# j4n1k/rl4co-slap

Hardware: AMD Instinct MI355X
Metric: env-steps/sec (batch×decode) SLAP & TSP-100 at 1/2/4/8 MI355X (higher is better)
Workload: dtype u8+i64+f32

## Files before the change

### rl4co_slap_amd/csrc/co_common.hpp

```cpp
#pragma once

#include <hip/hip_runtime.h>
#include <stdint.h>

#include "../../include/co_env.h"

namespace co {

constexpr int kWave = 64;

__device__ __forceinline__ int lane_id() { return threadIdx.x & (kWave - 1); }
__device__ __forceinline__ int wave_in_block() {
  return __builtin_amdgcn_readfirstlane(threadIdx.x >> 6);
}

template <typename T>
__device__ __forceinline__ T wave_sum(T v) {
#pragma unroll
  for (int off = 32; off > 0; off >>= 1) v += __shfl_xor(v, off, kWave);
  return v;
}

__device__ __forceinline__ float wave_max(float v) {
#pragma unroll
// ... 81 lines not shown
    const auto r = __builtin_amdgcn_permlane16_swap(v, v, false, false);
    v = op(r[0], r[1]);
  }
  if (RL >= 64) {
    const auto r = __builtin_amdgcn_permlane32_swap(v, v, false, false);
    v = op(r[0], r[1]);
  }
  return v;
}

template <int RL>
__device__ __forceinline__ double grp_sum_f64(double v) {
  uint32_t lo = (uint32_t)__double_as_longlong(v), hi = (uint32_t)(__double_as_longlong(v) >> 32);
  auto join = [](uint32_t l, uint32_t h) {
    return __longlong_as_double((long long)(((uint64_t)h << 32) | l));
  };
#define CO_DPP_F64(C)                                   \
  {                                                     \
    v = v + join(dpp_u<C>(lo), dpp_u<C>(hi));           \
    lo = (uint32_t)__double_as_longlong(v);             \
    hi = (uint32_t)(__double_as_longlong(v) >> 32);     \
  }
  if (RL >= 2) CO_DPP_F64(0xB1);
  if (RL >= 4) CO_DPP_F64(0x4E);
  if (RL >= 8) CO_DPP_F64(0x141);
  if (RL >= 16) CO_DPP_F64(0x140);
#undef CO_DPP_F64
  if (RL >= 32) {
    const auto rl = __builtin_amdgcn_permlane16_swap(lo, lo, false, false);
    const auto rh = __builtin_amdgcn_permlane16_swap(hi, hi, false, false);
    v = join(rl[0], rh[0]) + join(rl[1], rh[1]);
    lo = (uint32_t)__double_as_longlong(v);
    hi = (uint32_t)(__double_as_longlong(v) >> 32);
  }
  if (RL >= 64) {
    const auto rl = __builtin_amdgcn_permlane32_swap(lo, lo, false, false);
    const auto rh = __builtin_amdgcn_permlane32_swap(hi, hi, false, false);
    v = join(rl[0], rh[0]) + join(rl[1], rh[1]);
  }
  return v;
}

template <int RL>
__device__ __forceinline__ float grp_max(float v) {
  return __uint_as_float(grp_reduce<RL>(__float_as_uint(v), [](uint32_t x, uint32_t y) {
    return __float_as_uint(fmaxf(__uint_as_float(x), __uint_as_float(y)));
  }));
}
template <int RL>
__device__ __forceinline__ float grp_max_ord(float v) {
  const int b = __float_as_int(v);
  int o = b ^ ((b >> 31) & 0x7fffffff);
  o = (int)grp_reduce<RL>((uint32_t)o, [](uint32_t x, uint32_t y) {
    return (uint32_t)max((int)x, (int)y);
  });
  return __int_as_float(o ^ ((o >> 31) & 0x7fffffff));
}
template <int RL>
__device__ __forceinline__ float grp_sum(float v) {
  return __uint_as_float(grp_reduce<RL>(__float_as_uint(v), [](uint32_t x, uint32_t y) {
    return __float_as_uint(__uint_as_float(x) + __uint_as_float(y));
  }));
}
template <int RL>
__device__ __forceinline__ void grp_argmax(float& v, int& idx) {
  uint32_t uv = __float_as_uint(v), ui = (uint32_t)idx;
  grp_reduce2<RL>(uv, ui, [](uint32_t ov, uint32_t oi, uint32_t cv, uint32_t ci) {
    return argmax_better(__uint_as_float(ov), (int)oi, __uint_as_float(cv), (int)ci);
  });
  v = __uint_as_float(uv);
  idx = (int)ui;
}
template <int RL>
__device__ __forceinline__ int grp_min_int(int v) {
  return (int)grp_reduce<RL>((uint32_t)v, [](uint32_t x, uint32_t y) {
    return (uint32_t)min((int)x, (int)y);
  });
}
template <int RL>
__device__ __forceinline__ int grp_max_int(int v) {
  return (int)grp_reduce<RL>((uint32_t)v, [](uint32_t x, uint32_t y) {
    return (uint32_t)max((int)x, (int)y);
  });
}

template <int RL>
__device__ __forceinline__ void grp_argmin(float& v, int& idx) {
  uint32_t uv = __float_as_uint(v), ui = (uint32_t)idx;
  grp_reduce2<RL>(uv, ui, [](uint32_t ov, uint32_t oi, uint32_t cv, uint32_t ci) {
    const float a = __uint_as_float(ov), b = __uint_as_float(cv);
    return a < b || (a == b && (int)oi < (int)ci);
  });
  v = __uint_as_float(uv);
  idx = (int)ui;
}

template <int RL>
__device__ __forceinline__ void grp_argmin_split(float& v, int& idx) {
  const float m = __uint_as_float(grp_reduce<RL>(__float_as_uint(v), [](uint32_t a, uint32_t b) {
    return __float_as_uint(fminf(__uint_as_float(a), __uint_as_float(b)));
  }));
  const int cand = v == m ? idx : 0x7fffffff;
  idx = (int)grp_reduce<RL>((uint32_t)cand, [](uint32_t a, uint32_t b) {
    return (uint32_t)min((int)a, (int)b);
  });
  v = m;
}

struct StripMove {
  int i, j;
};

__device__ __forceinline__ StripMove strip_move(int q, int c, int n) {
  const int r = q + 1, a = n - r;
  const bool first = c < a;
  const int d = first ? r : n - 1 - r, t = first ? c : c - a;
  StripMove m;
  m.i = 1 + t;
  m.j = 1 + t + d;
  return m;
}

constexpr uint32_t kDistKeyInf = 0xff800000u;
__device__ __forceinline__ uint32_t dist_key(float d) {
  const uint32_t u = __float_as_uint(d + 0.0f);
  return u ^ ((uint32_t)((int32_t)u >> 31) | 0x80000000u);
}
__device__ __forceinline__ uint32_t key_sel32(uint64_t m, uint32_t t, uint32_t f) {
  uint32_t r;
  asm("v_cndmask_b32_e64 %0, %1, %2, %3" : "=v"(r) : "v"(f), "v"(t), "s"(m));
  return r;
}
__device__ __forceinline__ void key_cswap(uint64_t& a, uint64_t& b) {
  const uint64_t lt = __builtin_amdgcn_ballot_w64(a < b);
  const uint32_t alo = (uint32_t)a, ahi = (uint32_t)(a >> 32), blo = (uint32_t)b,
                 bhi = (uint32_t)(b >> 32);
  a = ((uint64_t)key_sel32(lt, ahi, bhi) << 32) | key_sel32(lt, alo, blo);
  b = ((uint64_t)key_sel32(lt, bhi, ahi) << 32) | key_sel32(lt, blo, alo);
}
template <int E>
__device__ __forceinline__ void sort_keys(uint64_t (&k)[E]) {
  static_assert((E & (E - 1)) == 0, "E must be a power of two");
#pragma unroll
  for (int p = 1; p < E; p <<= 1)
#pragma unroll
    for (int q = p; q > 0; q >>= 1)
#pragma unroll
      for (int j = q % p; j + q < E; j += 2 * q)
#pragma unroll
        for (int i = 0; i < q; ++i)
          if (i + j + q < E && (i + j) / (2 * p) == (i + j + q) / (2 * p))
            key_cswap(k[i + j], k[i + j + q]);
}

typedef __attribute__((address_space(3))) void lds_void;

template <int AUX = 0>
__device__ __forceinline__ void stage_bytes_lds(const unsigned char* __restrict__ src, int nbytes,
                                                unsigned char* dst) {
  const int lane = threadIdx.x & 63, wave = wave_in_block(), nw = blockDim.x >> 6;
  const int n16 = nbytes & ~15;
  for (int base = wave * 1024; base < n16; base += nw * 1024) {
    const int off = base + lane * 16;
    if (off < n16)
      __builtin_amdgcn_global_load_lds((const void*)(src + off), (lds_void*)(dst + base), 16, 0,
                                       AUX);
  }
  for (int k = n16 + (int)threadIdx.x; k < nbytes; k += blockDim.x) dst[k] = src[k];
  __builtin_amdgcn_s_waitcnt(0);
  __syncthreads();
}

template <int AUX = 0>
__device__ __forceinline__ void wave_dma(const unsigned char* __restrict__ src, int nbytes,
                                         unsigned char* dst) {
  const int lane = lane_id(), n16 = nbytes & ~15;
  for (int base = 0; base < n16; base += 1024) {
    if (base + lane * 16 < n16)
      __builtin_amdgcn_global_load_lds((const void*)(src + base + lane * 16),
                                       (lds_void*)(dst + base), 16, 0, AUX);
  }
  if (lane < ((nbytes - n16) >> 2))
    reinterpret_cast<uint32_t*>(dst + n16)[lane] = reinterpret_cast<const uint32_t*>(src + n16)[lane];
}

__device__ __forceinline__ void wave_dma_wait() {
  __builtin_amdgcn_s_waitcnt(0);
  __builtin_amdgcn_fence(__ATOMIC_RELEASE, "wavefront");
  __builtin_amdgcn_wave_barrier();
  __builtin_amdgcn_fence(__ATOMIC_ACQUIRE, "wavefront");
}

namespace {
__global__ void zero_i32_kernel(int32_t* p) { *p = 0; }
}
inline int zero_i32(int32_t* p, hipStream_t s) {
  hipLaunchKernelGGL(zero_i32_kernel, dim3(1), dim3(1), 0, s, p);
  return (int)hipGetLastError();
}

inline unsigned grid_for(int64_t work_items, int per_block, int64_t cap = 256 * 16) {
  int64_t g = (work_items + per_block - 1) / per_block;
  if (g < 1) g = 1;
  if (g > cap) g = cap;
  return (unsigned)g;
}

constexpr int64_t kMaxCoverThreads = ((int64_t)1 << 32) - 1;
inline unsigned cover_grid(int64_t work_items, int per_block, int block_threads = 256) {
  int64_t g = (work_items + per_block - 1) / per_block;
  if (g < 1) g = 1;
  if (g * (int64_t)block_threads > kMaxCoverThreads) return 0;
  return (unsigned)g;
}

inline int launch_status() {
  hipError_t e = hipGetLastError();
  return e == hipSuccess ? CO_OK : (int)e;
}

}

int co_internal_tsp_reward_stepmajor(int64_t B, int64_t N, const float* locs,
                                     int64_t locs_batch, const int64_t* acts, int64_t st,
                                     int check, float* reward, int32_t* status, void* stream);
int co_internal_tsp_reward_rows(int64_t B, int64_t N, const float* locs, int64_t locs_batch,
                                const int64_t* acts, int64_t sb, int check, float* reward,
                                int32_t* status, void* stream);
int co_internal_tsp_nearest_rollout(int64_t B, int64_t N, const float* locs, int64_t* acts_out,
                                    uint8_t* mask_out, int64_t* first_out, int64_t* cur_out,
                                    int64_t* i_out, uint8_t* done_out, uint8_t* step_reward_out,
                                    float* reward_out, void* stream);
```

### rl4co_slap_amd/csrc/co_diag.hpp

```cpp
#pragma once

namespace co {

#ifdef CO_DIAG_FASTTANH
constexpr bool kDiagFastTanh = true;
#else
constexpr bool kDiagFastTanh = false;
#endif

#ifdef CO_DIAG_FASTEXP
constexpr bool kDiagFastExp = true;
#else
constexpr bool kDiagFastExp = false;
#endif

#ifdef CO_DIAG_CERT_COUNT
constexpr bool kDiagCertCount = true;
#else
constexpr bool kDiagCertCount = false;
#endif

#ifdef CO_DIAG_CVRP_CUT
constexpr int kDiagCvrpCut = CO_DIAG_CVRP_CUT;
#else
constexpr int kDiagCvrpCut = 0;
#endif

constexpr bool kDiagTimingCut = kDiagFastTanh || kDiagFastExp || kDiagCvrpCut != 0;

}
```

### rl4co_slap_amd/csrc/decode_step.hip

```cpp
#include "decode_common.hpp"

#if defined(CO_DIAG_FASTTANH) || defined(CO_DIAG_FASTEXP) || defined(CO_DIAG_CVRP_CUT) || \
    defined(CO_DIAG_CERT_COUNT)
extern "C" __attribute__((visibility("default"))) const int co_variant_timing_cut_decode = 1;
#endif

extern "C" int co_decode_step_ex(int64_t B, int64_t N, const float* logits, int64_t lstride,
                                 const uint8_t* mask, float clip, float temp, int top_k,
                                 double top_p, int mode, const int64_t* action_in,
                                 int64_t* action_out, float* logp_sel, float* full, uint64_t seed,
                                 uint64_t offset, int32_t* status, void* stream) {
  if (B < 0 || N <= 0 || N > (1 << 24) || top_k < 0 || top_p < 0.0 || top_p > 1.0)
    return CO_E_INVAL;
  const bool cert = (mode & CO_DECODE_CERTIFIED) != 0 && (mode & CO_DECODE_FAST) == 0;
  const bool fast = (mode & CO_DECODE_FAST) != 0;
  mode &= ~(CO_DECODE_FAST | CO_DECODE_CERTIFIED);
  if (mode < 0 || mode > 2) return CO_E_MODE;
  if (B == 0) return CO_OK;
  if (!logits || !action_out) return CO_E_INVAL;
  if (mode == CO_DECODE_EVALUATE && !action_in) return CO_E_INVAL;
  hipStream_t s = (hipStream_t)stream;
  if (N > 64 * 32) {
    if (top_p > 0.0 && top_p < 1.0) return CO_E_INVAL;
    const dim3 lgrid((unsigned)(B < 65536 ? B : 65536)), lblock(kLongThreads);
    const int opt = (clip > 0.f ? kOptClip : 0) | (temp != 1.f ? kOptTemp : 0);
#define CO_LONG(O)                                                                             \
  hipLaunchKernelGGL(decode_long_kernel<O>, lgrid, lblock, 0, s, B, (int)N, logits, lstride,   \
                     mask, clip, temp, mode, action_in, action_out, logp_sel, full, seed, offset, \
                     status, top_k)
    switch (opt) {
      case 0: CO_LONG(0); break;
      case 1: CO_LONG(1); break;
      case 2: CO_LONG(2); break;
      default: CO_LONG(3);
    }
#undef CO_LONG
    return launch_status();
  }
  const dim3 grid(decode_grid(B, (int)N)), block(256);
  if (grid.x == 0) return CO_E_INVAL;
  const bool filtered = (top_k > 0 && top_k < N) || (top_p > 0.0 && top_p < 1.0);
  if (mode == CO_DECODE_GREEDY && !filtered) {
#define CO_GREEDY(RL, EPL, V)                                                                  \
  CO_OPT_DISPATCH_G(hipLaunchKernelGGL, (decode_greedy_kernel<RL, (EPL < 4 ? 4 : EPL), V, OPT>), \
                  grid, block, 0, s, B, (int)N, logits, lstride, mask, clip, temp, action_out,  \
                  logp_sel, full, status)
    switch (greedy_vw(N, lstride, logits, mask, mask, full)) {
      case 4: CO_ROW_DISPATCH(CO_GREEDY, 4); break;
      case 2: CO_GREEDY(CO_RL16, 16 / CO_RL16, 2); break;
      default: CO_ROW_DISPATCH(CO_GREEDY, 3);
    }
#undef CO_GREEDY
    return launch_status();
  }
#define CO_DECODE(RL, EPL, V)                                                                  \
  CO_OPT_DISPATCH(hipLaunchKernelGGL, (decode_kernel<RL, EPL, V, OPT>), grid, block, 0, s, B,   \
                  (int)N, logits, lstride, mask, clip, temp, mode, action_in, action_out,      \
                  logp_sel, full, seed, offset, status, top_k, top_p)
  if (decode_vec_ok(logits, lstride, mask, N)) {
    CO_ROW_DISPATCH(CO_DECODE, true);
  } else {
    CO_ROW_DISPATCH(CO_DECODE, false);
  }
#undef CO_DECODE
  return launch_status();
}

extern "C" int co_decode_step(int64_t B, int64_t N, const float* logits, int64_t lstride,
                              const uint8_t* mask, float clip, float temp, int mode,
                              const int64_t* action_in, int64_t* action_out, float* logp_sel,
                              float* full, uint64_t seed, uint64_t offset, int32_t* status,
                              void* stream) {
  return co_decode_step_ex(B, N, logits, lstride, mask, clip, temp, 0, 0.0, mode, action_in,
                           action_out, logp_sel, full, seed, offset, status, stream);
}

namespace {
__global__ __launch_bounds__(64) void beam_select_kernel(
    int64_t B, int BW, int N, const float* __restrict__ logp, int64_t lstride,
    const float* __restrict__ parent, const uint8_t* __restrict__ mask,
    int64_t* __restrict__ selected, int32_t* __restrict__ beam_parent,
    int64_t* __restrict__ beam_row, float* __restrict__ score_out, int32_t* status) {
  extern __shared__ __attribute__((aligned(16))) unsigned char smem[];
  const int T = BW * N;
  float* sc = reinterpret_cast<float*>(smem);
  uint32_t* taken = reinterpret_cast<uint32_t*>(sc + T);
  const int lane = threadIdx.x;
  for (int64_t b = blockIdx.x; b < B; b += gridDim.x) {
    for (int t = lane; t < T; t += 64) {
      const int s = t / N, c = t - s * N;
      const int64_t r = (int64_t)s * B + b;
      sc[t] = logp[r * lstride + c] + parent[r];
    }
    for (int w = lane; w < (T + 31) / 32; w += 64) taken[w] = 0u;
    __syncthreads();
    bool bad = false;
    for (int j = 0; j < BW; ++j) {
      float bv = -__builtin_inff();
      int bi = 0x7fffffff;
      for (int t = lane; t < T; t += 64) {
        const bool free_t = !((taken[t >> 5] >> (t & 31)) & 1u);
        const float v = sc[t];
        if (free_t && (bi == 0x7fffffff || argmax_better(v, t, bv, bi))) {
          bv = v;
          bi = t;
        }
      }
      wave_argmax(bv, bi);
      if (bi == 0x7fffffff) bi = 0;
      const int s = bi / N, c = bi - s * N;
      if (lane == 0) {
        taken[bi >> 5] |= 1u << (bi & 31);
        const int64_t row = (int64_t)j * B + b;
        selected[row] = c;
        beam_parent[row] = s;
        beam_row[row] = b + (int64_t)s * B;
        score_out[row] = bv;
        if (mask && !mask[(b + (int64_t)s * B) * N + c]) bad = true;
      }
      __syncthreads();
    }
    if (bad) set_status(status, CO_ST_INFEASIBLE);
    __syncthreads();
  }
}
}

extern "C" int co_beam_select(int64_t B, int64_t BW, int64_t N, const float* logp,
                              int64_t lstride, const float* parent, const uint8_t* mask,
                              int64_t* selected, int32_t* beam_parent, int64_t* beam_row,
                              float* score_out, int32_t* status, void* stream) {
  if (B < 0 || BW <= 0 || N <= 0 || BW > N * BW || BW * N > 36 * 1024) return CO_E_INVAL;
  if (B == 0) return CO_OK;
  if (!logp || !parent || !selected || !beam_parent || !beam_row || !score_out ||
      (mask && !status))
    return CO_E_INVAL;
  const int T = (int)(BW * N);
  const size_t shmem = (size_t)T * 4 + (size_t)((T + 31) / 32) * 4;
  if (shmem > 64 * 1024)
    (void)hipFuncSetAttribute((const void*)beam_select_kernel,
                              hipFuncAttributeMaxDynamicSharedMemorySize, (int)shmem);
  hipLaunchKernelGGL(beam_select_kernel, dim3((unsigned)(B < 65536 ? B : 65536)), dim3(64),
                     shmem, (hipStream_t)stream, B, (int)BW, (int)N, logp, lstride, parent,
                     mask, selected, beam_parent, beam_row, score_out, status);
  return launch_status();
}
```

### rl4co_slap_amd/csrc/rollout.hip

```cpp
#include "co_common.hpp"

using namespace co;

namespace {


inline int NW_launch(int64_t n) {
  const int w = (int)((n + 63) / 64);
  return w <= 1 ? 1 : (w == 2 ? 2 : 4);
}

template <int NW>
__device__ __forceinline__ void mask_row_to_lds(const uint64_t (&m)[NW], int n,
                                                unsigned char* row, int c_lo = 0,
                                                int c_hi = -1) {
  if (c_hi < 0) c_hi = n;
  if ((n & 3) == 0 && (c_lo & 3) == 0) {
    for (int c = c_lo; c < c_hi; c += 4) {
      uint32_t v = 0;
#pragma unroll
      for (int j = 0; j < 4; ++j) {
        const int cc = c + j;
        uint64_t w = 0;
#pragma unroll
        for (int k = 0; k < NW; ++k)
          if ((cc >> 6) == k) w = m[k];
        v |= (uint32_t)((w >> (cc & 63)) & 1ull) << (8 * j);
      }
      *reinterpret_cast<uint32_t*>(row + c) = v;
    }
  } else {
    for (int c = c_lo; c < c_hi; ++c) {
      uint64_t w = 0;
#pragma unroll
      for (int k = 0; k < NW; ++k)
        if ((c >> 6) == k) w = m[k];
      row[c] = (unsigned char)((w >> (c & 63)) & 1ull);
    }
  }
}

__device__ __forceinline__ void copy_tile_out(const unsigned char* scratch, int nbytes,
                                              uint8_t* __restrict__ dst) {
  const int tid = threadIdx.x;
  const int n16 = ((reinterpret_cast<uintptr_t>(dst) & 15) == 0) ? (nbytes & ~15) : 0;
  for (int off = tid * 16; off < n16; off += blockDim.x * 16)
    *reinterpret_cast<uint4*>(dst + off) = *reinterpret_cast<const uint4*>(scratch + off);
  for (int k = n16 + tid; k < nbytes; k += blockDim.x) dst[k] = scratch[k];
}

__device__ __forceinline__ void zero_tile_out(int nbytes, uint8_t* __restrict__ dst) {
  const int tid = threadIdx.x;
  const int n16 = ((reinterpret_cast<uintptr_t>(dst) & 15) == 0) ? (nbytes & ~15) : 0;
  for (int off = tid * 16; off < n16; off += blockDim.x * 16)
    *reinterpret_cast<uint4*>(dst + off) = make_uint4(0u, 0u, 0u, 0u);
  for (int k = n16 + tid; k < nbytes; k += blockDim.x) dst[k] = 0;
}

__host__ __device__ inline size_t tsp_tile_bytes(int N, int Q) {
  const size_t xy = (size_t)64 * N * 8;
  const size_t scr = (((size_t)64 * N + 15) & ~(size_t)15) + (size_t)Q * 64 * 8 + 64 * 8 + 64 * 4 +
                     16 * 4;
  return ((xy > scr ? xy : scr) + 15) & ~(size_t)15;
}

#ifndef CO_TEACH_Q
#define CO_TEACH_Q 4
#endif
#ifndef CO_TEACH_U
#define CO_TEACH_U 8
#endif
template <int NW, int Q, bool STATE, int NB = 0>
__global__ __launch_bounds__(64 * Q) void tsp_teacher_kernel(
    int64_t B, int N, const float2* __restrict__ locs, int64_t LB,
    const int64_t* __restrict__ acts_in, uint8_t* __restrict__ mask_out,
    int64_t* __restrict__ first_out, int64_t* __restrict__ cur_out, int64_t* __restrict__ i_out,
    uint8_t* __restrict__ done_out, uint8_t* __restrict__ step_reward_out,
    float* __restrict__ reward_out, int check, int32_t* status) {
  extern __shared__ __attribute__((aligned(16))) unsigned char smem[];
  float2* s_xy = reinterpret_cast<float2*>(smem);
  constexpr int VS = 2 * NW + 1;
  uint32_t* s_vis = reinterpret_cast<uint32_t*>(smem + tsp_tile_bytes(N, Q));
  const int lane = threadIdx.x & 63, q = wave_in_block();
  const int64_t row0 = (int64_t)blockIdx.x * 64;
  const int rows = (int)((B - row0) < 64 ? (B - row0) : 64);
  const int64_t b = row0 + lane;
  const bool live = lane < rows;

  const int R = (N - 1 + Q - 1) / Q;
  const int t_lo = 1 + q * R < N ? 1 + q * R : N;
  const int t_hi = t_lo + R < N ? t_lo + R : N;
  constexpr int U = CO_TEACH_U;
  int64_t bufA[U], bufB[U];
  const int64_t* ap = acts_in + (live ? b : row0);
  auto load = [&](int64_t (&dst)[U], int t0) {
    const int tc = t0 + U <= t_hi ? t0 : t_hi - U;
    const int64_t* p = ap + (int64_t)tc * B;
#pragma unroll
    for (int u = 0; u < U; ++u) {
      dst[u] = *p;
      p += B;
    }
  };
  const int nfull = (t_hi - t_lo) / U;
  const int64_t a_prev = ap[(int64_t)(q == 0 ? 0 : t_lo - 1) * B];
  if (nfull > 0) load(bufA, t_lo);
  if (q == 0) {
    for (int k = 0; k < NW; ++k) {
      const int lo = k * 64;
      const uint64_t w = (N >= lo + 64) ? ~0ull : (N > lo ? ((1ull << (N - lo)) - 1ull) : 0ull);
      s_vis[lane * VS + 2 * k] = (uint32_t)w;
      s_vis[lane * VS + 2 * k + 1] = (uint32_t)(w >> 32);
    }
  }
  stage_bytes_lds(reinterpret_cast<const unsigned char*>(locs + (row0 % LB) * N), rows * N * 8,
                  reinterpret_cast<unsigned char*>(s_xy));
  const float2* xy = s_xy + lane * N;
  uint32_t* vw = s_vis + lane * VS;
  uint32_t badw = 0;
  int a = 0;
  float px = 0.f, py = 0.f, fx = 0.f, fy = 0.f;
  double len = 0.0;
  if (live) {
    const uint32_t lo = (uint32_t)a_prev;
    const uint32_t in = ((uint32_t)(a_prev >> 32) == 0u) & (lo < (uint32_t)N);
    a = in ? (int)lo : 0;
    if (q == 0) {
      badw |= in ^ 1u;
      __hip_atomic_fetch_and(&vw[a >> 5], ~(1u << (a & 31)), __ATOMIC_RELAXED,
                             __HIP_MEMORY_SCOPE_WORKGROUP);
    }
    const float2 p0 = xy[a];
    px = fx = p0.x;
    py = fy = p0.y;
    auto run = [&](const int64_t (&src)[U], int cnt) {
      int av[U];
#pragma unroll
      for (int u = 0; u < U; ++u) {
        if (u < cnt) {
          const uint32_t l32 = (uint32_t)src[u];
          const uint32_t ok = ((uint32_t)(src[u] >> 32) == 0u) & (l32 < (uint32_t)N);
          badw |= ok ^ 1u;
          av[u] = ok ? (int)l32 : 0;
        }
      }
      float2 qq[U];
#pragma unroll
      for (int u = 0; u < U; ++u)
        if (u < cnt) qq[u] = xy[av[u]];
#pragma unroll
      for (int u = 0; u < U; ++u)
        if (u < cnt)
          __hip_atomic_fetch_and(&vw[av[u] >> 5], ~(1u << (av[u] & 31)), __ATOMIC_RELAXED,
// ... 150 lines not shown
#pragma unroll
      for (int k = 0; k < EPL; k += 2) {
        if (valid && t0 + k + 1 < N) {
          const longlong2 v = *reinterpret_cast<const longlong2*>(arow + t0 + k);
          av[k] = v.x;
          av[k + 1] = v.y;
        } else {
          av[k] = (valid && t0 + k < N) ? arow[t0 + k] : 0;
          av[k + 1] = 0;
        }
      }
    } else {
#pragma unroll
      for (int k = 0; k < EPL; ++k) av[k] = (valid && t0 + k < N) ? arow[t0 + k] : 0;
    }
    for (int j = sl; j < NWB; j += G) bits[j] = 0u;
    uint32_t bad = 0;
    int node[EPL];
#pragma unroll
    for (int k = 0; k < EPL; ++k) {
      const uint32_t l32 = (uint32_t)av[k];
      const bool ok = ((uint32_t)(av[k] >> 32) == 0u) & (l32 < (uint32_t)N);
      const bool in = t0 + k < N;
      bad |= (in && !ok) ? 1u : 0u;
      node[k] = ok ? (int)l32 : 0;
    }
    const float2* lrow = DMA ? s_xy + grp * N : locs + (LB == B ? rr : rr % LB) * (int64_t)N;
    float2 p[EPL];
    if constexpr (DMA) {
#pragma unroll
      for (int k = 0; k < EPL; ++k) p[k] = lrow[node[k]];
    } else {
#pragma unroll
      for (int k = 0; k < EPL; ++k)
        p[k] = (valid && t0 + k < N) ? lrow[node[k]] : make_float2(0.f, 0.f);
    }
    __builtin_amdgcn_fence(__ATOMIC_RELEASE, "wavefront");
    __builtin_amdgcn_wave_barrier();
    __builtin_amdgcn_fence(__ATOMIC_ACQUIRE, "wavefront");
#pragma unroll
    for (int k = 0; k < EPL; ++k)
      __hip_atomic_fetch_or(&bits[node[k] >> 5],
                            (valid && t0 + k < N) ? 1u << (node[k] & 31) : 0u, __ATOMIC_RELAXED,
                            __HIP_MEMORY_SCOPE_WAVEFRONT);
    double acc = 0.0;
#pragma unroll
    for (int k = 1; k < EPL; ++k) {
      const float dx = p[k].x - p[k - 1].x, dy = p[k].y - p[k - 1].y;
      const float e = __builtin_amdgcn_sqrtf(dx * dx + dy * dy);
      acc += t0 + k < N ? (double)e : 0.0;
    }
    const float nx = __shfl_down(p[0].x, 1, G), ny = __shfl_down(p[0].y, 1, G);
    const float fx = __shfl(p[0].x, 0, G), fy = __shfl(p[0].y, 0, G);
    const int tl = N - 1 - t0;
    float lx = p[EPL - 1].x, ly = p[EPL - 1].y;
#pragma unroll
    for (int k = 0; k < EPL - 1; ++k)
      if (k == tl) {
        lx = p[k].x;
        ly = p[k].y;
      }
    {
      const bool cross = t0 + EPL < N, closing = !cross && tl >= 0 && tl < EPL;
      const float tx = cross ? nx : fx, ty = cross ? ny : fy;
      const float dx = tx - lx, dy = ty - ly;
      const float e = __builtin_amdgcn_sqrtf(dx * dx + dy * dy);
      acc += (cross || closing) ? (double)e : 0.0;
    }
    const float len = (float)grp_sum_f64<G>(acc);
    __builtin_amdgcn_fence(__ATOMIC_RELEASE, "wavefront");
    __builtin_amdgcn_wave_barrier();
    __builtin_amdgcn_fence(__ATOMIC_ACQUIRE, "wavefront");
    int cnt = 0;
    for (int j = sl; j < nwords; j += G) cnt += __popc(bits[j]);
    cnt = (int)grp_reduce<G>((uint32_t)cnt, [](uint32_t x, uint32_t y) { return x + y; });
    bad = grp_reduce<G>(bad, [](uint32_t x, uint32_t y) { return x | y; });
    const bool full = cnt == N;
    if (check && valid && sl == 0 && (bad || !full)) set_status(status, CO_ST_INVALID_TOUR);
    if (!valid) return;
    if constexpr (STATE) {
      uint8_t* mrow = mask_out + r * (int64_t)N;
      const bool wide = ((reinterpret_cast<uintptr_t>(mrow) | (uintptr_t)N) & 3) == 0;
      if (wide) {
        for (int c4 = sl; c4 < (N >> 2); c4 += G) {
          uint32_t v = 0;
          if (!full) {
            const uint32_t nib = ~(bits[c4 >> 3] >> (4 * (c4 & 7))) & 0xfu;
            v = (nib & 1u) | ((nib & 2u) << 7) | ((nib & 4u) << 14) | ((nib & 8u) << 21);
          }
          __builtin_nontemporal_store(v, reinterpret_cast<uint32_t*>(mrow + 4 * c4));
        }
      } else {
        for (int c = sl; c < N; c += G)
          mrow[c] = full ? 0 : (uint8_t)(((bits[c >> 5] >> (c & 31)) & 1u) ^ 1u);
      }
      const int last_lane = (N - 1) / EPL;
      int lastnode = node[0];
#pragma unroll
      for (int k = 0; k < EPL; ++k)
        if (k == tl) lastnode = node[k];
      if (sl == 0) {
        first_out[r] = node[0];
        i_out[r] = N;
        reward_out[r] = -(float)len;
      }
      if (sl == last_lane) cur_out[r] = lastnode;
      if (sl == (G > 2 ? 2 : 1) % G) {
        done_out[r] = full;
        step_reward_out[r] = 0;
      }
    } else {
      if (sl == 0) reward_out[r] = -(float)len;
    }
  }
}

__device__ __forceinline__ float edge_len_hw(float x0, float y0, float x1, float y1) {
  const float dx = x1 - x0, dy = y1 - y0;
  return __builtin_amdgcn_sqrtf(dx * dx + dy * dy);
}
__device__ __forceinline__ int slap_pick_loc(int pp, const int32_t* asg, int L, bool& range) {
  const bool neg = pp < 0;
  int64_t loc = asg[neg ? 0 : pp];
  loc = loc < 0 ? loc + L : loc;
  const bool bad = neg || loc < 0 || loc >= L;
  range |= bad;
  return bad ? 0 : (int)loc;
}
template <int KU, typename PK>
__device__ __forceinline__ float slap_order_len(const PK* pk, const int32_t* asg,
                                                const float2* xy, int L, bool& range,
                                                int K = KU) {
  int pp[KU], lc[KU];
  float2 q[KU];
#pragma unroll
  for (int k = 0; k < KU; ++k) pp[k] = k < K ? pk[k] : 0;
#pragma unroll
  for (int k = 0; k < KU; ++k) lc[k] = k < K ? slap_pick_loc(pp[k], asg, L, range) : 0;
#pragma unroll
  for (int k = 0; k < KU; ++k) q[k] = xy[lc[k]];
  float len = 0.f;
#pragma unroll
  for (int k = 1; k < KU; ++k)
    if (k < K) len += edge_len_hw(q[k - 1].x, q[k - 1].y, q[k].x, q[k].y);
  float2 ql = q[0];
#pragma unroll
  for (int k = 1; k < KU; ++k) ql = (k == K - 1) ? q[k] : ql;
  return len + edge_len_hw(ql.x, ql.y, q[0].x, q[0].y);
}

__host__ __device__ inline size_t slap_asg_bytes(int ipb, int P) {
  return ((size_t)ipb * P * 4 + 15) & ~(size_t)15;
}
__host__ __device__ inline size_t slap_wave_bytes(int gpw, int epl, int L, int O, int K) {
  const size_t keys = (size_t)epl * 64 * 8;
  const size_t data = (size_t)gpw * (L * 8 + O * 4 + O * K * 2);
  return ((keys > data ? keys : data) + 15) & ~(size_t)15;
}
__host__ __device__ inline size_t slap_xy_bytes(int gpw, int L) {
  return ((size_t)gpw * L * 8 + 15) & ~(size_t)15;
}
__host__ __device__ inline size_t slap_wave_bytes_sd(int gpw, int epl, int L, int O, int K) {
  size_t area = (size_t)(epl - 2) * 64 * 8;
  const size_t dd = (size_t)gpw * L * 4, tail = (size_t)gpw * (O * 4 + O * K * 2);
  area = area > dd ? area : dd;
  area = area > tail ? area : tail;
  return slap_xy_bytes(gpw, L) + ((area + 15) & ~(size_t)15);
}

__device__ __forceinline__ float2 ld_pair(const float2* p) { return *p; }

template <int G, int EPL, bool CLOSEST, bool SD>
__global__ __launch_bounds__(256) void slap_group_kernel(
    int64_t B, int L, int P, int O, int K, const float2* __restrict__ locs,
    const int64_t* __restrict__ picklist, const float* __restrict__ depot_dist,
    const int32_t* __restrict__ assign_in, const int64_t* __restrict__ acts_in,
    int64_t* __restrict__ acts_out, uint8_t* __restrict__ mask_out,
    int32_t* __restrict__ assign_out, int64_t* __restrict__ i_out, uint8_t* __restrict__ done_out,
    uint8_t* __restrict__ step_reward_out, float* __restrict__ reward_out,
    float* __restrict__ ratio_out, int32_t* status) {
  constexpr int IPB = 256 / G, GPW = 64 / G;
  extern __shared__ __attribute__((aligned(16))) unsigned char smem[];
  const int lane = lane_id(), sl = lane % G, g = threadIdx.x / G, gw = lane / G;
  int32_t* s_asg = reinterpret_cast<int32_t*>(smem);
  unsigned char* wreg =
      smem + slap_asg_bytes(IPB, P) +
      (size_t)wave_in_block() * (SD ? slap_wave_bytes_sd(GPW, EPL, L, O, K)
                                    : slap_wave_bytes(GPW, EPL, L, O, K));
  unsigned char* area = wreg + (SD ? slap_xy_bytes(GPW, L) : 0);
  uint64_t* s_keys = reinterpret_cast<uint64_t*>(area) - (SD ? 2 * 64 : 0);
  const int64_t b = (int64_t)blockIdx.x * IPB + g;
  const bool live = b < B;
  const int64_t bb = live ? b : 0;
  float2* xy = reinterpret_cast<float2*>(wreg) + gw * L;
  int32_t* asg = s_asg + g * P;
  unsigned char* obase = SD ? area : wreg + (size_t)GPW * L * 8;
  float* olen = reinterpret_cast<float*>(obase) + gw * O;
  int16_t* pks = reinterpret_cast<int16_t*>(obase + (size_t)GPW * O * 4) + gw * O * K;
  const int64_t wbase = (int64_t)blockIdx.x * IPB + (int64_t)wave_in_block() * GPW;
  const int wrows = (int)(B - wbase < GPW ? (B - wbase > 0 ? B - wbase : 0) : GPW);
  if constexpr (SD) {
    wave_dma<2>(reinterpret_cast<const unsigned char*>(depot_dist + wbase * L), wrows * L * 4,
                area);
    wave_dma_wait();
  }

  float dd[EPL];
  uint32_t avail = 0;
#pragma unroll
  for (int k = 0; k < EPL; ++k) {
    const int c = sl + G * k;
    const bool ok = c < L && c != 0;
    if (ok) avail |= 1u << k;
    if constexpr (SD)
      dd[k] = (CLOSEST && ok) ? reinterpret_cast<const float*>(area)[gw * L + c] : __builtin_inff();
    else
      dd[k] = (CLOSEST && ok) ? (depot_dist + bb * L)[c] : __builtin_inff();
  }
  if constexpr (SD) {
    __builtin_amdgcn_s_waitcnt(0xc07f);
    wave_dma<2>(reinterpret_cast<const unsigned char*>(locs + wbase * L), wrows * L * 8, wreg);
  }
  if (live && ratio_out) {
    float* rrow = ratio_out + bb * L;
    if (((reinterpret_cast<uintptr_t>(ratio_out) | ((uintptr_t)L * 4)) & 15) == 0) {
      for (int c4 = sl; c4 < (L >> 2); c4 += G)
        *reinterpret_cast<float4*>(rrow + 4 * c4) = make_float4(0.f, 0.f, 0.f, 0.f);
    } else {
      for (int c = sl; c < L; c += G) rrow[c] = 0.f;
    }
  }
  const float2* lrow = locs + bb * L;
  const int64_t* prow = picklist + bb * (int64_t)O * K;
  float2 xr[EPL];
  int64_t pr[EPL];
#pragma unroll
  for (int k = 0; k < EPL; ++k) {
    const int c = sl + G * k;
    if constexpr (!SD) xr[k] = c < L ? ld_pair(lrow + c) : make_float2(0.f, 0.f);
    pr[k] = c < O * K ? prow[c] : 0;
  }
  auto wrap_product = [&](int64_t pp) -> int32_t {
    if (pp < 0) pp += P;
    return (pp < 0 || pp >= P) ? -1 : (int32_t)pp;
  };
  int32_t pw[EPL];
#pragma unroll
  for (int k = 0; k < EPL; ++k) pw[k] = wrap_product(pr[k]);
  uint64_t key[EPL];
  if (CLOSEST) {
#pragma unroll
    for (int k = 0; k < EPL; ++k)
      key[k] = ((uint64_t)dist_key(dd[k]) << 32) | (uint32_t)(sl + G * k);
    sort_keys<EPL>(key);
  }
  bool range = false;
  if (CLOSEST) {
    uint64_t hk = key[0], nk = EPL > 1 ? key[1] : ~0ull;
#pragma unroll
    for (int k = 2; k < EPL; ++k) s_keys[k * 64 + lane] = key[k];
    int h = 2;
    for (int t = 0; t < P; ++t) {
      const uint32_t hh = (uint32_t)(hk >> 32);
      const uint32_t gm = grp_reduce<G>(hh, [](uint32_t x, uint32_t y) { return x < y ? x : y; });
      const uint32_t cand = hh == gm ? (uint32_t)hk : 0xffffffffu;
      const uint32_t gi =
          grp_reduce<G>(cand, [](uint32_t x, uint32_t y) { return x < y ? x : y; });
      const bool any = gm < kDistKeyInf;
      if (any && (uint32_t)hk == gi) {
        avail &= ~(1u << (gi / G));
        hk = nk;
        nk = h < EPL ? s_keys[h * 64 + lane] : ~0ull;
        ++h;
      }
      if (sl == 0) asg[t] = any ? (int32_t)gi : 0;
    }
  } else {
    int32_t* s_w = reinterpret_cast<int32_t*>(wreg) + gw * P;
    if (P * GPW <= EPL * 128) {
#pragma unroll 4
      for (int t = sl; t < P; t += G) {
        const int64_t a64 = acts_in[(int64_t)t * B + bb];
        asg[t] = (int32_t)a64;
        const int64_t a = a64 < 0 ? a64 + L : a64;
        const bool bad = a < 0 || a >= L;
        range |= bad;
        s_w[t] = bad ? -1 : (int)a;
      }
      __builtin_amdgcn_fence(__ATOMIC_RELEASE, "wavefront");
      __builtin_amdgcn_wave_barrier();
      __builtin_amdgcn_fence(__ATOMIC_ACQUIRE, "wavefront");
      for (int t = 0; t < P; ++t) {
        const int a = s_w[t];
        if (a >= 0 && sl == a % G) avail &= ~(1u << (a / G));
      }
    } else {
      for (int t = 0; t < P; ++t) {
        const int64_t a64 = acts_in[(int64_t)t * B + bb];
        if (sl == 0) asg[t] = (int32_t)a64;
        const int64_t a = a64 < 0 ? a64 + L : a64;
        if (a < 0 || a >= L) {
          range = true;
        } else if (sl == (int)(a % G)) {
          avail &= ~(1u << (int)(a / G));
        }
      }
    }
  }
  if constexpr (SD) {
    __builtin_amdgcn_s_waitcnt(0);
  } else {
#pragma unroll
    for (int k = 0; k < EPL; ++k) {
      const int c = sl + G * k;
      if (c < L) xy[c] = xr[k];
    }
  }
#pragma unroll
  for (int k = 0; k < EPL; ++k) {
    const int c = sl + G * k;
    if (c < O * K) pks[c] = (int16_t)pw[k];
  }
  for (int c = sl + G * EPL; c < O * K; c += G) pks[c] = (int16_t)wrap_product(prow[c]);
  __builtin_amdgcn_fence(__ATOMIC_RELEASE, "wavefront");
  __builtin_amdgcn_wave_barrier();
  __builtin_amdgcn_fence(__ATOMIC_ACQUIRE, "wavefront");

  if (CLOSEST) {
    constexpr int IPW = 64 / G;
    const int w0 = wave_in_block() * IPW;
    for (int idx = lane; idx < IPW * P; idx += 64) {
      const int t = idx / IPW, gi = idx - t * IPW;
      const int64_t be = (int64_t)blockIdx.x * IPB + w0 + gi;
      if (be < B) {
        int64_t* dst = acts_out + (int64_t)t * B + be;
        *dst = (int64_t)s_asg[(w0 + gi) * P + t];
      }
    }
  }
  for (int o = sl; o < O; o += G) {
    const int16_t* pk = pks + o * K;
    float len = 0.f;
    if (K == 5) {
      len = slap_order_len<5>(pk, asg, xy, L, range);
    } else if (K <= 8) {
      len = slap_order_len<8>(pk, asg, xy, L, range, K);
    } else {
      float2 p0 = make_float2(0.f, 0.f), prev = p0;
      for (int k = 0; k < K; ++k) {
        const float2 q = xy[slap_pick_loc(pk[k], asg, L, range)];
        if (k == 0) {
          p0 = q;
        } else {
          len += edge_len_hw(prev.x, prev.y, q.x, q.y);
        }
        prev = q;
      }
      len += edge_len_hw(prev.x, prev.y, p0.x, p0.y);
    }
    olen[o] = len;
  }
  __builtin_amdgcn_fence(__ATOMIC_RELEASE, "wavefront");
  __builtin_amdgcn_wave_barrier();
  __builtin_amdgcn_fence(__ATOMIC_ACQUIRE, "wavefront");

  if (live) {
    uint8_t* mrow = mask_out + bb * L;
    if (((reinterpret_cast<uintptr_t>(mask_out) | (uintptr_t)L) & 3) == 0) {
      uint8_t* sm = reinterpret_cast<uint8_t*>(xy);
#pragma unroll
      for (int k = 0; k < EPL; ++k) {
        const int c = sl + G * k;
        if (c < L) sm[c] = (uint8_t)((avail >> k) & 1u);
      }
      __builtin_amdgcn_fence(__ATOMIC_RELEASE, "wavefront");
      __builtin_amdgcn_wave_barrier();
      __builtin_amdgcn_fence(__ATOMIC_ACQUIRE, "wavefront");
      for (int d = sl; d < (L >> 2); d += G)
        *reinterpret_cast<uint32_t*>(mrow + 4 * d) = *reinterpret_cast<const uint32_t*>(sm + 4 * d);
    } else {
#pragma unroll
      for (int k = 0; k < EPL; ++k) {
        const int c = sl + G * k;
        if (c < L) {
          uint8_t* dst = mrow + c;
          *dst = (uint8_t)((avail >> k) & 1u);
        }
      }
    }
    if (((reinterpret_cast<uintptr_t>(assign_out) | ((uintptr_t)P * 4)) & 15) == 0) {
      for (int c4 = sl; c4 < (P >> 2); c4 += G)
        *reinterpret_cast<int4*>(assign_out + bb * P + 4 * c4) =
            *reinterpret_cast<const int4*>(asg + 4 * c4);
    } else {
#pragma unroll 2
      for (int c = sl; c < P; c += G) {
        int32_t* dst = assign_out + bb * P + c;
        *dst = asg[c];
      }
    }
    if (sl == 0) {
      float total = 0.f;
      int o = 0;
      if ((O & 3) == 0 && (reinterpret_cast<uintptr_t>(olen) & 15) == 0)
        for (; o < O; o += 4) {
          const float4 v = *reinterpret_cast<const float4*>(olen + o);
          total += -v.x;
          total += -v.y;
          total += -v.z;
          total += -v.w;
        }
      for (; o < O; ++o) total += -olen[o];
      reward_out[bb] = total;
      i_out[bb] = P;
      done_out[bb] = 1;
      step_reward_out[bb] = 0;
    }
  }
  if (__any(range && live) && lane == 0) set_status(status, CO_ST_INDEX_RANGE);
}


template <bool STATE>
int launch_tsp_teacher(int64_t B, int64_t N, const float2* l2, int64_t LB, const int64_t* acts,
                       uint8_t* mask_out, int64_t* first_out, int64_t* cur_out, int64_t* i_out,
                       uint8_t* done_out, uint8_t* step_reward_out, float* reward_out, int check,
                       int32_t* status, hipStream_t s) {
  constexpr int Q = CO_TEACH_Q;
  const int NW = NW_launch(N);
  const size_t shmem = tsp_tile_bytes((int)N, Q) + (size_t)64 * (2 * NW + 1) * 4;
  const dim3 grid(cover_grid(B, 64, 64 * Q)), block(64 * Q);
  if (grid.x == 0) return CO_E_INVAL;
#define CO_TEACH(W)                                                                            \
  do {                                                                                         \
    if (shmem > 64 * 1024)                                                                     \
      (void)hipFuncSetAttribute((const void*)tsp_teacher_kernel<W, Q, STATE, 0>,               \
                                hipFuncAttributeMaxDynamicSharedMemorySize, (int)shmem);       \
    hipLaunchKernelGGL((tsp_teacher_kernel<W, Q, STATE, 0>), grid, block, shmem, s, B, (int)N, \
                       l2, LB, acts, mask_out, first_out, cur_out, i_out, done_out,                \
                       step_reward_out, reward_out, check, status);                            \
  } while (0)
  if (NW == 1) CO_TEACH(1);
  else if (NW == 2) CO_TEACH(2);
  else CO_TEACH(4);
#undef CO_TEACH
  return launch_status();
}

template <bool STATE>
int launch_tsp_rows(int64_t B, int64_t N, const float2* l2, int64_t LB, const int64_t* acts,
                    int64_t sb, uint8_t* mask_out, int64_t* first_out, int64_t* cur_out,
                    int64_t* i_out, uint8_t* done_out, uint8_t* step_reward_out,
                    float* reward_out, int check, int32_t* status, hipStream_t s) {
  const bool vec = ((reinterpret_cast<uintptr_t>(acts) & 15) == 0) && (sb % 2 == 0);
  const bool dma_ok = sb == N &&
                      ((reinterpret_cast<uintptr_t>(acts) | reinterpret_cast<uintptr_t>(l2)) & 15) == 0;
#define CO_ROWS(GG, EE)                                                                        \
  do {                                                                                         \
    constexpr int WPB = CO_ROWS_WPB;                                                           \
    const dim3 grid(cover_grid((B + 64 / GG - 1) / (64 / GG), WPB, 64 * WPB)), block(64 * WPB); \
    if (grid.x == 0) return CO_E_INVAL;                                                        \
    const size_t dsh = WPB * tsp_rows_wave_bytes(64 / GG, (int)N);                             \
           \
    const size_t sbits = (size_t)WPB * (64 / GG) * ((GG * EE + 31) / 32) * 4;                  \
    if (dma_ok && (LB == B || LB % (64 / GG) == 0) && dsh + sbits <= 64 * 1024)                \
      hipLaunchKernelGGL((tsp_teacher_rows_kernel<GG, EE, 3, STATE>), grid, block, dsh, s, B,   \
                         (int)N, l2, LB, acts, sb, mask_out, first_out, cur_out, i_out,        \
                         done_out, step_reward_out, reward_out, check, status);                \
    else if (vec)                                                                              \
      hipLaunchKernelGGL((tsp_teacher_rows_kernel<GG, EE, 1, STATE>), grid, block, 0, s, B,     \
                         (int)N, l2, LB, acts, sb, mask_out, first_out, cur_out, i_out,        \
                         done_out, step_reward_out, reward_out, check, status);                \
    else                                                                                       \
      hipLaunchKernelGGL((tsp_teacher_rows_kernel<GG, EE, 0, STATE>), grid, block, 0, s, B,     \
                         (int)N, l2, LB, acts, sb, mask_out, first_out, cur_out, i_out,        \
                         done_out, step_reward_out, reward_out, check, status);                \
  } while (0)
  if (N <= 32) CO_ROWS(4, 8);
  else if (N <= 64) CO_ROWS(8, 8);
  else if (N <= 16 * CO_ROWS_EPL112) CO_ROWS(16, CO_ROWS_EPL112);
  else if (N <= 128) CO_ROWS(16, 8);
  else if (N <= 256) CO_ROWS(32, 8);
  else if (N <= 512) CO_ROWS(64, 8);
  else CO_ROWS(64, 16);
#undef CO_ROWS
  return launch_status();
}

}

int co_internal_tsp_reward_rows(int64_t B, int64_t N, const float* locs, int64_t locs_batch,
                                const int64_t* acts, int64_t sb, int check, float* reward,
                                int32_t* status, void* stream) {
  if (N > 1024 || sb < N || (reinterpret_cast<uintptr_t>(locs) & 7)) return CO_E_INVAL;
  return launch_tsp_rows<false>(B, N, reinterpret_cast<const float2*>(locs), locs_batch, acts, sb,
                                nullptr, nullptr, nullptr, nullptr, nullptr, nullptr, reward,
                                check, status, (hipStream_t)stream);
}

namespace {
int tsp_rollout_stepwise(int64_t B, int64_t N, const float* locs, const int64_t* acts_in,
                         int64_t* acts_out, uint8_t* mask_out, int64_t* first_out,
                         int64_t* cur_out, int64_t* i_out, uint8_t* done_out,
                         uint8_t* step_reward_out, float* reward_out, int check, int32_t* status,
                         void* stream) {
  int rc = co_tsp_reset(B, N, mask_out, first_out, cur_out, i_out, reward_out, stream);
  const bool nearest = acts_in == nullptr;
  const int64_t* acts = nearest ? acts_out : acts_in;
  for (int64_t t = 0; t < N && rc == CO_OK; ++t) {
    if (nearest)
      rc = co_tsp_nearest_action(B, N, locs, mask_out, cur_out, t == 0, acts_out + t * B,
                                 stream);
    if (rc == CO_OK)
      rc = co_tsp_step(B, N, acts + t * B, mask_out, mask_out, i_out, i_out, first_out,
                       first_out, cur_out, done_out, step_reward_out, t == 0 ? 1 : 0, nullptr,
                       status, stream);
  }
  if (rc != CO_OK) return rc;
  return co_tsp_reward(B, N, N, locs, B, acts, 1, B, check, reward_out, status, stream);
}
}

extern "C" int co_tsp_rollout_ex(int64_t B, int64_t N, const float* locs,
                                 const int64_t* acts_in, int64_t sb, int64_t st,
                                 int64_t* acts_out, uint8_t* mask_out, int64_t* first_out,
                                 int64_t* cur_out, int64_t* i_out, uint8_t* done_out,
                                 uint8_t* step_reward_out, float* reward_out, int check,
                                 int32_t* status, void* stream) {
  if (B < 0 || N <= 0 || N > (1 << 24)) return CO_E_INVAL;
  if (B == 0) return CO_OK;
  const bool nearest = acts_in == nullptr;
  if (!locs || !mask_out || !first_out || !cur_out || !i_out || !done_out || !step_reward_out ||
      !reward_out || (nearest && !acts_out) || (check && !status))
    return CO_E_INVAL;
  if (reinterpret_cast<uintptr_t>(locs) & 7) return CO_E_ALIGN;
  if (!nearest && !(sb == 1 && st == B)) {
    if (st != 1 || sb < N || N > 1024) return CO_E_INVAL;
    return launch_tsp_rows<true>(B, N, reinterpret_cast<const float2*>(locs), B, acts_in, sb,
                                 mask_out, first_out, cur_out, i_out, done_out, step_reward_out,
                                 reward_out, check, status, (hipStream_t)stream);
  }
  if (N > (nearest ? 1024 : 256))
    return tsp_rollout_stepwise(B, N, locs, acts_in, acts_out, mask_out, first_out, cur_out,
                                i_out, done_out, step_reward_out, reward_out, check, status,
                                stream);
  if (nearest)
    return co_internal_tsp_nearest_rollout(B, N, locs, acts_out, mask_out, first_out, cur_out,
                                           i_out, done_out, step_reward_out, reward_out, stream);
  if (reinterpret_cast<uintptr_t>(locs) & 15) return CO_E_ALIGN;
  return launch_tsp_teacher<true>(B, N, reinterpret_cast<const float2*>(locs), B, acts_in,
                                  mask_out,
                                  first_out, cur_out, i_out, done_out, step_reward_out,
                                  reward_out, check, status, (hipStream_t)stream);
}

extern "C" int co_tsp_rollout(int64_t B, int64_t N, const float* locs, const int64_t* acts_in,
                              int64_t* acts_out, uint8_t* mask_out, int64_t* first_out,
                              int64_t* cur_out, int64_t* i_out, uint8_t* done_out,
                              uint8_t* step_reward_out, float* reward_out, int check,
                              int32_t* status, void* stream) {
  return co_tsp_rollout_ex(B, N, locs, acts_in, 1, B, acts_out, mask_out, first_out, cur_out,
                           i_out, done_out, step_reward_out, reward_out, check, status, stream);
}

int co_internal_tsp_reward_stepmajor(int64_t B, int64_t N, const float* locs,
                                     int64_t locs_batch, const int64_t* acts, int64_t st,
                                     int check, float* reward, int32_t* status, void* stream) {
  if (st != B || N > 256 || (reinterpret_cast<uintptr_t>(locs) & 15)) return CO_E_INVAL;
  if (locs_batch != B && locs_batch % 64 != 0) return CO_E_INVAL;
  return launch_tsp_teacher<false>(B, N, reinterpret_cast<const float2*>(locs), locs_batch, acts,
                                   nullptr,
                                   nullptr, nullptr, nullptr, nullptr, nullptr, reward, check,
                                   status, (hipStream_t)stream);
}

extern "C" int co_slap_rollout(int64_t B, int64_t L, int64_t P, int64_t O, int64_t K,
                               const float* locs, const int64_t* picklist,
                               const float* depot_dist, const int32_t* assign_in,
                               const int64_t* acts_in, int64_t* acts_out, uint8_t* mask_out,
                               int32_t* assign_out, int64_t* i_out, uint8_t* done_out,
                               uint8_t* step_reward_out, float* reward_out, float* ratio_out,
                               int32_t* status, void* stream) {
  if (B < 0 || L <= 1 || L > 256 || P <= 0 || O <= 0 || K <= 0 || P > 4096) return CO_E_INVAL;
  if (B == 0) return CO_OK;
  const bool closest = acts_in == nullptr;
  if (!locs || !picklist || !assign_in || !mask_out || !assign_out || !i_out || !done_out ||
      !step_reward_out || !reward_out || !status || (closest && (!acts_out || !depot_dist)))
    return CO_E_INVAL;
  if (reinterpret_cast<uintptr_t>(locs) & 7) return CO_E_ALIGN;
  const int G = L <= 64 ? 8 : (L <= 128 ? 16 : 32);
  const int ipb = 256 / G;
  const bool sd = closest && (L % 4) == 0 &&
                  ((reinterpret_cast<uintptr_t>(locs) | reinterpret_cast<uintptr_t>(depot_dist)) &
                   15) == 0;
  const size_t shmem =
      slap_asg_bytes(ipb, (int)P) +
      4 * (sd ? slap_wave_bytes_sd(64 / G, 8, (int)L, (int)O, (int)K)
              : slap_wave_bytes(64 / G, 8, (int)L, (int)O, (int)K));
  if (shmem > 160 * 1024) return CO_E_INVAL;
  const dim3 grid(cover_grid(B, ipb)), block(256);
  if (grid.x == 0) return CO_E_INVAL;
  hipStream_t s = (hipStream_t)stream;
  const float2* l2 = reinterpret_cast<const float2*>(locs);
#define CO_SLAP(GG, EPL, C, SDD)                                                               \
  do {                                                                                         \
    if (shmem > 64 * 1024)                                                                     \
      (void)hipFuncSetAttribute((const void*)slap_group_kernel<GG, EPL, C, SDD>,               \
                                hipFuncAttributeMaxDynamicSharedMemorySize, (int)shmem);       \
    hipLaunchKernelGGL((slap_group_kernel<GG, EPL, C, SDD>), grid, block, shmem, s, B, (int)L, \
                       (int)P, (int)O, (int)K, l2, picklist, depot_dist, assign_in, acts_in,   \
                       acts_out, mask_out, assign_out, i_out, done_out, step_reward_out,       \
                       reward_out, ratio_out, status);                                         \
  } while (0)
#define CO_SLAP_G(C, SDD)                                       \
  if (G == 8) CO_SLAP(8, 8, C, SDD);                            \
  else if (G == 16) CO_SLAP(16, 8, C, SDD);                     \
  else CO_SLAP(32, 8, C, SDD)
  if (closest && sd) {
    CO_SLAP_G(true, true);
  } else if (closest) {
    CO_SLAP_G(true, false);
  } else {
    CO_SLAP_G(false, false);
  }
#undef CO_SLAP_G
#undef CO_SLAP
  return launch_status();
}
```

Baseline: 352.2 billion.

## Pack SLAP closest-location keys into 32-bit registers with exact tie fallback

The closest-assignment path of the SLAP kernel now packs distance and location index into one 32-bit key by overwriting the low distance bits with the location id. It sorts these keys in registers and drops the LDS-spilled 64-bit key stream, so each step needs only one group min-reduction instead of two. Because truncating distance bits can reorder near-ties, the kernel checks whether any truncated ties occurred and whether the resulting order breaks the exact ordering. If so, it reruns the original 64-bit selection. This also removes the key scratch area from shared memory, which shrinks the per-wave LDS footprint, and adds a diagnostic macro that flags fallback runs.

```diff
diff --git a/rl4co_slap_amd/csrc/co_common.hpp b/rl4co_slap_amd/csrc/co_common.hpp
--- a/rl4co_slap_amd/csrc/co_common.hpp
+++ b/rl4co_slap_amd/csrc/co_common.hpp
@@ -257,6 +257,23 @@
           if (i + j + q < E && (i + j) / (2 * p) == (i + j + q) / (2 * p))
             key_cswap(k[i + j], k[i + j + q]);
 }
+template <int E>
+__device__ __forceinline__ void sort_keys32(uint32_t (&k)[E]) {
+  static_assert((E & (E - 1)) == 0, "E must be a power of two");
+#pragma unroll
+  for (int p = 1; p < E; p <<= 1)
+#pragma unroll
+    for (int q = p; q > 0; q >>= 1)
+#pragma unroll
+      for (int j = q % p; j + q < E; j += 2 * q)
+#pragma unroll
+        for (int i = 0; i < q; ++i)
+          if (i + j + q < E && (i + j) / (2 * p) == (i + j + q) / (2 * p)) {
+            const uint32_t lo = min(k[i + j], k[i + j + q]), hi = max(k[i + j], k[i + j + q]);
+            k[i + j] = lo;
+            k[i + j + q] = hi;
+          }
+}
 
 typedef __attribute__((address_space(3))) void lds_void;
 
diff --git a/rl4co_slap_amd/csrc/co_diag.hpp b/rl4co_slap_amd/csrc/co_diag.hpp
--- a/rl4co_slap_amd/csrc/co_diag.hpp
+++ b/rl4co_slap_amd/csrc/co_diag.hpp
@@ -26,6 +26,12 @@
 constexpr int kDiagCvrpCut = 0;
 #endif
 
+#ifdef CO_DIAG_SLAP_FALLBACK
+constexpr bool kDiagSlapFallback = true;
+#else
+constexpr bool kDiagSlapFallback = false;
+#endif
+
 constexpr bool kDiagTimingCut = kDiagFastTanh || kDiagFastExp || kDiagCvrpCut != 0;
 
 }
diff --git a/rl4co_slap_amd/csrc/decode_step.hip b/rl4co_slap_amd/csrc/decode_step.hip
--- a/rl4co_slap_amd/csrc/decode_step.hip
+++ b/rl4co_slap_amd/csrc/decode_step.hip
@@ -1,7 +1,7 @@
 #include "decode_common.hpp"
 
 #if defined(CO_DIAG_FASTTANH) || defined(CO_DIAG_FASTEXP) || defined(CO_DIAG_CVRP_CUT) || \
-    defined(CO_DIAG_CERT_COUNT)
+    defined(CO_DIAG_CERT_COUNT) || defined(CO_DIAG_SLAP_FALLBACK)
 extern "C" __attribute__((visibility("default"))) const int co_variant_timing_cut_decode = 1;
 #endif
 
diff --git a/rl4co_slap_amd/csrc/rollout.hip b/rl4co_slap_amd/csrc/rollout.hip
--- a/rl4co_slap_amd/csrc/rollout.hip
+++ b/rl4co_slap_amd/csrc/rollout.hip
@@ -1,4 +1,5 @@
 #include "co_common.hpp"
+#include "co_diag.hpp"
 
 using namespace co;
 
@@ -455,19 +456,18 @@
 __host__ __device__ inline size_t slap_asg_bytes(int ipb, int P) {
   return ((size_t)ipb * P * 4 + 15) & ~(size_t)15;
 }
-__host__ __device__ inline size_t slap_wave_bytes(int gpw, int epl, int L, int O, int K) {
-  const size_t keys = (size_t)epl * 64 * 8;
+__host__ __device__ inline size_t slap_wave_bytes(int gpw, int epl, int L, int O, int K,
+                                                  bool closest) {
+  const size_t keys = closest ? 0 : (size_t)epl * 64 * 8;
   const size_t data = (size_t)gpw * (L * 8 + O * 4 + O * K * 2);
   return ((keys > data ? keys : data) + 15) & ~(size_t)15;
 }
 __host__ __device__ inline size_t slap_xy_bytes(int gpw, int L) {
   return ((size_t)gpw * L * 8 + 15) & ~(size_t)15;
 }
-__host__ __device__ inline size_t slap_wave_bytes_sd(int gpw, int epl, int L, int O, int K) {
-  size_t area = (size_t)(epl - 2) * 64 * 8;
+__host__ __device__ inline size_t slap_wave_bytes_sd(int gpw, int L, int O, int K) {
   const size_t dd = (size_t)gpw * L * 4, tail = (size_t)gpw * (O * 4 + O * K * 2);
-  area = area > dd ? area : dd;
-  area = area > tail ? area : tail;
+  const size_t area = dd > tail ? dd : tail;
   return slap_xy_bytes(gpw, L) + ((area + 15) & ~(size_t)15);
 }
 
@@ -488,10 +488,9 @@
   int32_t* s_asg = reinterpret_cast<int32_t*>(smem);
   unsigned char* wreg =
       smem + slap_asg_bytes(IPB, P) +
-      (size_t)wave_in_block() * (SD ? slap_wave_bytes_sd(GPW, EPL, L, O, K)
-                                    : slap_wave_bytes(GPW, EPL, L, O, K));
+      (size_t)wave_in_block() * (SD ? slap_wave_bytes_sd(GPW, L, O, K)
+                                    : slap_wave_bytes(GPW, EPL, L, O, K, CLOSEST));
   unsigned char* area = wreg + (SD ? slap_xy_bytes(GPW, L) : 0);
-  uint64_t* s_keys = reinterpret_cast<uint64_t*>(area) - (SD ? 2 * 64 : 0);
   const int64_t b = (int64_t)blockIdx.x * IPB + g;
   const bool live = b < B;
   const int64_t bb = live ? b : 0;
@@ -550,34 +549,94 @@
   int32_t pw[EPL];
 #pragma unroll
   for (int k = 0; k < EPL; ++k) pw[k] = wrap_product(pr[k]);
-  uint64_t key[EPL];
+  bool range = false;
+  [[maybe_unused]] bool diag_redo = false;
   if (CLOSEST) {
+    constexpr uint32_t kLocMask = (uint32_t)(G * EPL - 1);
+    static_assert((G * EPL & (G * EPL - 1)) == 0 && G * EPL <= 256, "location bits");
+    const float* drow = depot_dist + bb * L;
+    uint32_t key[EPL];
 #pragma unroll
     for (int k = 0; k < EPL; ++k)
-      key[k] = ((uint64_t)dist_key(dd[k]) << 32) | (uint32_t)(sl + G * k);
-    sort_keys<EPL>(key);
-  }
-  bool range = false;
-  if (CLOSEST) {
-    uint64_t hk = key[0], nk = EPL > 1 ? key[1] : ~0ull;
-#pragma unroll
-    for (int k = 2; k < EPL; ++k) s_keys[k * 64 + lane] = key[k];
-    int h = 2;
+      key[k] = (dist_key(dd[k]) & ~kLocMask) | (uint32_t)(sl + G * k);
+    sort_keys32<EPL>(key);
+    uint32_t gprev = ~0u;
+    bool tied = false;
     for (int t = 0; t < P; ++t) {
-      const uint32_t hh = (uint32_t)(hk >> 32);
-      const uint32_t gm = grp_reduce<G>(hh, [](uint32_t x, uint32_t y) { return x < y ? x : y; });
-      const uint32_t cand = hh == gm ? (uint32_t)hk : 0xffffffffu;
-      const uint32_t gi =
-          grp_reduce<G>(cand, [](uint32_t x, uint32_t y) { return x < y ? x : y; });
+      const uint32_t gm =
+          grp_reduce<G>(key[0], [](uint32_t x, uint32_t y) { return x < y ? x : y; });
       const bool any = gm < kDistKeyInf;
-      if (any && (uint32_t)hk == gi) {
-        avail &= ~(1u << (gi / G));
-        hk = nk;
-        nk = h < EPL ? s_keys[h * 64 + lane] : ~0ull;
-        ++h;
-      }
-      if (sl == 0) asg[t] = any ? (int32_t)gi : 0;
-    }
+      tied |= any && (gm ^ gprev) <= kLocMask;
+      gprev = gm;
+      if (any && key[0] == gm) {
+        avail &= ~(1u << ((gm & kLocMask) / G));
+#pragma unroll
+        for (int k = 0; k + 1 < EPL; ++k) key[k] = key[k + 1];
+        key[EPL - 1] = ~0u;
+      }
+      if (sl == 0) asg[t] = any ? (int32_t)(gm & kLocMask) : 0;
+    }
+    tied |= gprev < kDistKeyInf && (key[0] ^ gprev) <= kLocMask;
+    bool viol = false;
+    if (__any(tied && live)) {
+      uint32_t* s_fk = reinterpret_cast<uint32_t*>(area) + gw * L;
+      uint32_t fk[EPL];
+#pragma unroll
+      for (int k = 0; k < EPL; ++k) {
+        const int c = sl + G * k;
+        const bool ok = c < L && c != 0;
+        fk[k] = dist_key(ok ? drow[c] : __builtin_inff());
+        if (c < L) s_fk[c] = fk[k];
+      }
+      __builtin_amdgcn_fence(__ATOMIC_RELEASE, "wavefront");
+      __builtin_amdgcn_wave_barrier();
+      __builtin_amdgcn_fence(__ATOMIC_ACQUIRE, "wavefront");
+#pragma unroll 1
+      for (int t = sl + 1; t < P; t += G) {
+        const uint32_t lp = (uint32_t)asg[t - 1], lc = (uint32_t)asg[t];
+        const uint64_t kp = ((uint64_t)s_fk[lp] << 32) | lp;
+        const uint64_t kc = ((uint64_t)s_fk[lc] << 32) | lc;
+        viol |= lc != 0 && kc <= kp;
+      }
+      const uint32_t ll = (uint32_t)asg[P - 1];
+      const uint64_t kl = ((uint64_t)s_fk[ll] << 32) | ll;
+#pragma unroll
+      for (int k = 0; k < EPL; ++k) {
+        const uint64_t kc = ((uint64_t)fk[k] << 32) | (uint32_t)(sl + G * k);
+        viol |= ll != 0 && ((avail >> k) & 1u) && kc < kl;
+      }
+    }
+    const bool redo = __any(viol && live);
+    if (redo) {
+      uint64_t key64[EPL];
+      avail = 0;
+#pragma unroll
+      for (int k = 0; k < EPL; ++k) {
+        const int c = sl + G * k;
+        const bool ok = c < L && c != 0;
+        if (ok) avail |= 1u << k;
+        const float d = ok ? drow[c] : __builtin_inff();
+        key64[k] = ((uint64_t)dist_key(d) << 32) | (uint32_t)c;
+      }
+      sort_keys<EPL>(key64);
+      for (int t = 0; t < P; ++t) {
+        const uint32_t hh = (uint32_t)(key64[0] >> 32);
+        const uint32_t g0 =
+            grp_reduce<G>(hh, [](uint32_t x, uint32_t y) { return x < y ? x : y; });
+        const uint32_t cand = hh == g0 ? (uint32_t)key64[0] : 0xffffffffu;
+        const uint32_t gi =
+            grp_reduce<G>(cand, [](uint32_t x, uint32_t y) { return x < y ? x : y; });
+        const bool any = g0 < kDistKeyInf;
+        if (any && (uint32_t)key64[0] == gi) {
+          avail &= ~(1u << (gi / G));
+#pragma unroll
+          for (int k = 0; k + 1 < EPL; ++k) key64[k] = key64[k + 1];
+          key64[EPL - 1] = ~0ull;
+        }
+        if (sl == 0) asg[t] = any ? (int32_t)gi : 0;
+      }
+    }
+    if (co::kDiagSlapFallback && redo) diag_redo = true;
   } else {
     int32_t* s_w = reinterpret_cast<int32_t*>(wreg) + gw * P;
     if (P * GPW <= EPL * 128) {
@@ -714,6 +773,7 @@
           total += -v.w;
         }
       for (; o < O; ++o) total += -olen[o];
+      if (co::kDiagSlapFallback && diag_redo) total = -12345.f;
       reward_out[bb] = total;
       i_out[bb] = P;
       done_out[bb] = 1;
@@ -898,8 +958,8 @@
                    15) == 0;
   const size_t shmem =
       slap_asg_bytes(ipb, (int)P) +
-      4 * (sd ? slap_wave_bytes_sd(64 / G, 8, (int)L, (int)O, (int)K)
-              : slap_wave_bytes(64 / G, 8, (int)L, (int)O, (int)K));
+      4 * (sd ? slap_wave_bytes_sd(64 / G, (int)L, (int)O, (int)K)
+              : slap_wave_bytes(64 / G, 8, (int)L, (int)O, (int)K, closest));
   if (shmem > 160 * 1024) return CO_E_INVAL;
   const dim3 grid(cover_grid(B, ipb)), block(256);
   if (grid.x == 0) return CO_E_INVAL;
```

Result: no change. 351.1 billion (-0.3%).
